# schumacherlab/ONT-TCRconsensus

Hardware: AMD Instinct MI355X
Metric: UMIs clustered/sec + banded-NW GCUPS (whole node, 1/2/4/8 MI355X) (higher is better)
Workload: dtype int16/int32

## Files before the change

### ont-tcrconsensus_amd/csrc/cluster_ctx.h

```cpp
#pragma once
#include <hip/hip_runtime.h>

#include <atomic>
#include <cstdlib>
#include <cstring>
#include <memory>
#include <thread>
#include <utility>
#include <vector>

#include "ctx.h"
#include "plan.h"
#include "resolve.h"

struct umiclust_ctx;

namespace uc {

constexpr int32_t kDelta = 8192;
constexpr int32_t kDepth = 2;
constexpr int32_t kBlockMin = 2048;
constexpr int32_t kDirectRecQ = 4096;
constexpr int32_t kSpecThr = 30;
constexpr int32_t kLazyPermille = 5;
// ... 15 lines not shown
struct Tile {
  DevBuf<uint32_t> hist;
  DevBuf<uint32_t> off;
  DevBuf<uint32_t> cursor;
  DevBuf<uint32_t> partial;
  uint64_t post_base = 0;
  size_t post_cap = 0;
  int32_t n = 0;
  int32_t base = 0;
  int32_t seg = 0;
  int32_t len = 0;
  int32_t built_n = -1;
  bool prebuilt = false;
};

struct Pass {
  int32_t q0 = 0, nq = 0, w0 = 0;
  bool live = false;
  bool rec_direct = false;
  PinBuf<TileView> h_tiles;
  DevBuf<TileView> d_tiles;
  DevBuf<uint32_t> d_top_seqno;
  DevBuf<uint8_t> d_top_count, d_ntop;
  DevBuf<uint32_t> d_pcand, d_units;
  DevBuf<uint8_t> d_pncand, d_ppeer_count, d_pnpeer;
  DevBuf<uint32_t> d_ppost;
  DevBuf<uint16_t> d_ppeer_id;
  DevBuf<uint16_t> d_peer_id;
  DevBuf<uint8_t> d_peer_count, d_npeer;
  bool ctr_zeroed = false;
  DevBuf<uint32_t> d_counters;
  DevBuf<uint32_t> d_pq, d_pt, d_outidx, d_res;
  DevBuf<WalkState> d_ws;
  DevBuf<HostQs> d_hq;
  DevBuf<unsigned long long> d_paligned;
  DevBuf<uint32_t> d_reccount;
  DevBuf<uint32_t> d_rec;
  uint32_t rec_est = 1u << 16;
  PinBuf<HostQs> h_hq;
  PinBuf<uint32_t> h_rec, h_counters, h_reccount;
  std::vector<HostQs> hq_copy;
  std::vector<uint32_t> rec_copy;
  ResolveScratch rsx;
  Event ev[5];
  PinBuf<TileView> h_tiles_a;
  DevBuf<TileView> d_tiles_a;
  DevBuf<uint32_t> d_anunits;
  Event ev_a;
  Event ev_c[2];
  bool c_timed = false;
  bool a_live = false, a_timed = false;
  int32_t a_q0 = -1, a_base = 0, a_slot = 0, t_slot = 0;
};

struct PfCapture {
  uint32_t* h_nunits = nullptr;
  int32_t ntiles = 0, nseg = 0, one_wave = 0;
};

struct Index {
  umiclust_ctx* const c;
  std::vector<std::unique_ptr<Tile>> tiles;
  Tile base_tile, delta_tile[2];
  int32_t delta_cur = 0;
  int32_t sealed_end = 0, base_end = 0;
  int32_t index_end = 0;
  DevBuf<uint16_t> arena;
  uint64_t sealed_slot0 = 0;
  std::vector<int32_t> cent;
  std::vector<uint8_t> cent_len;
  DevBuf<int32_t> d_cent;
  DevBuf<uint8_t> d_cent_len;
  PinBuf<int32_t> h_cent;
// ... 275 lines not shown
```

### ont-tcrconsensus_amd/csrc/kernels.hip

```cpp
#include <hip/hip_runtime.h>

#include <atomic>
#include <cstring>
#include <type_traits>
#include <mutex>

#include "align_kernels.h"
#include "umiclust_internal.h"

namespace uc {

enum { k_attr_prefilter = 0, k_attr_consensus = 1, k_attr_count = 2 };
constexpr int kAttrDevices = 64;
static std::atomic<bool> g_attr_set[kAttrDevices][k_attr_count];
static bool attr_set_on_device(int which) {
  int d = 0;
  if (hipGetDevice(&d) != hipSuccess || d < 0 || d >= kAttrDevices) return false;
  return g_attr_set[d][which];
}
static void mark_attr_set(int which) {
  int d = 0;
  if (hipGetDevice(&d) == hipSuccess && d >= 0 && d < kAttrDevices) g_attr_set[d][which] = true;
}

// ... 1398 lines not shown
                        int32_t band_max) {
  init_align_tables();
  if (npairs <= 0) return hipSuccess;
  if (qlen < kMinTplLen || qlen > kMaxLen) return hipErrorInvalidValue;
  const bool band = !ambig && npairs <= band_max;
  const int64_t lanes = (int64_t)npairs * (band ? band_lanes(qlen) : 1);
  const int v = ambig ? 1 : band ? 2 : 0;
  int64_t grid = (lanes + 63) / 64;
  hipLaunchKernelGGL(g_align[kAlignSlots * qlen + v], dim3((unsigned)grid),
                     dim3(64), 0, st, s, pq, pt, npairs, dev_npairs, outidx, sc, out);
  return hipGetLastError();
}

__device__ __forceinline__ uint32_t seg_alloc(uint32_t n, uint32_t si, uint32_t* cnt) {
  uint32_t start = 0;
  unsigned long long pending = __ballot(n > 0u);
  while (pending) {
    const int lead = __builtin_ctzll(pending);
    const uint32_t L = (uint32_t)__builtin_amdgcn_readlane((int)si, lead);
    const bool mine = n > 0u && si == L;
    const unsigned long long grp = __ballot(mine);
    const uint32_t v = mine ? n : 0u;
    const uint32_t incl = wave_scan_dpp(v, OpAdd());
    const uint32_t tot = lane63(incl);
    uint32_t b = 0;
    if ((int)(threadIdx.x & 63) == lead) b = atomicAdd(cnt + L, tot);
    b = (uint32_t)__builtin_amdgcn_readlane((int)b, lead);
    if (mine) start = b + incl - v;
    pending &= ~grp;
  }
  return start;
}

__global__ __launch_bounds__(256) void k_walk(int32_t round, int32_t q0, int32_t nqs, int32_t both, int32_t spec_thr,
                                              const uint32_t* __restrict__ top_seqno, const uint8_t* __restrict__ top_count,
                                              const uint8_t* __restrict__ ntop, const uint8_t* __restrict__ lens,
                                              const uint32_t* __restrict__ res, const uint8_t* __restrict__ acc_tab,
                                              const uint16_t* __restrict__ rank_tab, WalkState* __restrict__ ws,
                                              uint32_t* __restrict__ pq, uint32_t* __restrict__ pt,
                                              uint32_t* __restrict__ outidx, SegTab sg, uint32_t* __restrict__ seg_cnt,
                                              unsigned long long* __restrict__ cells) {
  const int qs = blockIdx.x * blockDim.x + threadIdx.x;
  const bool live = qs < nqs;
  const int32_t q = q0 + (live ? qs : 0) / both;
  const uint32_t strand = (uint32_t)((live ? qs : 0) % both);
  const int nt = live ? ntop[qs] : 0;
  const int ql = lens[q];
  WalkState w{};
  bool act = live;
  int emit_to = 0;
  if (round < 0) {
    w.w = 0;
    w.done = (nt == 0) ? 1 : 0;
    w.acc = 0;
    w.best_rank = 0;
    w.best_t = 0xffffffffu;
    w.cells = 0;
    w.lastkey = 0;
    w.e = 0;
    const bool spec = nt > 0 && (int)top_count[(int64_t)(live ? qs : 0) * kTopHits] < spec_thr;
    emit_to = min(nt, spec ? kWalk : kBatch);
  } else if (live) {
    w = ws[qs];
    act = !w.done;
    if (act) {
      while (!w.done && w.w < w.e) {
        const int b0 = w.w, b1 = min(nt, b0 + kBatch);
        for (int x = b0; x < b1; x++) {
          const uint32_t r = res[(int64_t)qs * kWalk + x];
          const uint32_t m = r & 0xffu, L = (r >> 8) & 0xffu;
          const uint32_t t = top_seqno[(int64_t)qs * kTopHits + x];
          w.cells += (uint32_t)(ql * lens[t]);
          if (acc_tab[L * kTabM + m]) {
            const uint16_t rk = rank_tab[L * kTabM + m];
            if (!w.acc || rk > w.best_rank || (rk == w.best_rank && t < w.best_t)) {
              w.best_rank = rk;
              w.best_t = t;
            }
            w.acc = 1;
          }
        }
        w.w = (uint8_t)b1;
        const uint32_t tl = lens[top_seqno[(int64_t)qs * kTopHits + b1 - 1]];
        w.lastkey = ((unsigned long long)(127u - top_count[(int64_t)qs * kTopHits + b1 - 1]) << 56) |
                    ((unsigned long long)tl << 48) | top_seqno[(int64_t)qs * kTopHits + b1 - 1];
        if (w.acc || b1 >= nt || b1 >= kWalk) w.done = 1;
      }
      emit_to = w.done ? (int)w.e : min(nt, kWalk);
    }
  }
  const uint32_t n = (act && emit_to > (int)w.e) ? (uint32_t)(emit_to - (int)w.e) : 0u;
  const uint32_t si = (uint32_t)(sg.lmax - ql);
  const uint32_t k0 = seg_alloc(n, si, seg_cnt);
  if (n) {
    const int b0 = w.e, b1 = emit_to;
    const uint32_t base = sg.base[si] + k0;
    uint32_t tl = 0;
    for (int x = b0; x < b1; x++) {
      const uint32_t k = base + (uint32_t)(x - b0);
      const uint32_t t = top_seqno[(int64_t)qs * kTopHits + x];
      pq[k] = ((uint32_t)q << 1) | strand;
      pt[k] = t;
      outidx[k] = (uint32_t)qs * kWalk + (uint32_t)x;
      tl += lens[t];
    }
    atomicAdd(cells, (unsigned long long)ql * tl);
    w.e = (uint8_t)b1;
  }
  if (act) ws[qs] = w;
}

hipError_t launch_walk(int32_t round, int32_t q0, int32_t nqs, int32_t both, int32_t spec_thr,
                       const uint32_t* top_seqno, const uint8_t* top_count, const uint8_t* ntop,
                       const uint8_t* lens, const uint32_t* res, const uint8_t* acc_tab,
                       const uint16_t* rank_tab, WalkState* ws, uint32_t* pq, uint32_t* pt,
                       uint32_t* outidx, const SegTab& sg, uint32_t* seg_cnt, unsigned long long* cells,
                       hipStream_t st) {
  if (nqs <= 0) return hipSuccess;
  hipLaunchKernelGGL(k_walk, dim3((nqs + 255) / 256), dim3(256), 0, st, round, q0, nqs, both, spec_thr,
                     top_seqno, top_count, ntop, lens, res, acc_tab, rank_tab, ws, pq, pt, outidx,
// ... 92 lines not shown
  atomicAdd(nstat, n);
  uint32_t k = sg.base[si] + k0;
  const uint32_t qv = ((uint32_t)q << 1) | (uint32_t)(qs % both);
  uint32_t tl = 0;
  for (int hh = 0; hh < kPH; hh++)
    for (unsigned long long m = rel[hh]; m; m &= m - 1ull) {
      const int x = 64 * hh + __builtin_ctzll(m);
      const uint32_t t = (uint32_t)(w0 + peer_id[(int64_t)qs * kPeerCap + x]);
      pq[k] = qv;
      pt[k] = t;
      outidx[k] = out0 + (uint32_t)(qs * kPeerCap + x);
      tl += lens[t];
      k++;
    }
  atomicAdd(cells, (unsigned long long)ql * tl);
}

hipError_t launch_peer_pairs(int32_t q0, int32_t w0, int32_t nqs, int32_t both, const uint8_t* lens,
                             const WalkState* ws, const uint16_t* peer_id, const uint8_t* peer_count,
                             const uint8_t* npeer, uint32_t* pq, uint32_t* pt, uint32_t* outidx, const SegTab& sg,
                             uint32_t* seg_cnt, unsigned long long* cells, uint32_t* nstat, uint32_t out0,
                             unsigned long long* aligned, int32_t emit, const WalkState* ws_prev,
                             const uint8_t* npeer_prev, int32_t q0_prev, int32_t nq_prev, hipStream_t st) {
  if (nqs <= 0) return hipSuccess;
  hipLaunchKernelGGL(k_peer_rel, dim3((nqs + 3) / 4), dim3(256), 0, st, q0, w0, nqs, both, lens, ws, peer_id,
                     peer_count, npeer, aligned, emit, ws_prev, npeer_prev, q0_prev, nq_prev);
  hipLaunchKernelGGL(k_peer_pairs, dim3((nqs + 255) / 256), dim3(256), 0, st, q0, w0, nqs, both, lens, ws, peer_id,
                     peer_count, npeer, pq, pt, outidx, sg, seg_cnt, cells, nstat, out0, aligned, emit, ws_prev,
                     npeer_prev, q0_prev, nq_prev);
  return hipGetLastError();
}

constexpr int kPackWaves = 4, kPackQ = 4;
__global__ __launch_bounds__(64 * kPackWaves) void k_pack(int32_t nqs, int32_t w0, const uint8_t* __restrict__ lens,
                                              const WalkState* __restrict__ ws, const uint8_t* __restrict__ ntop,
                                              const uint32_t* __restrict__ top_seqno,
                                              const uint8_t* __restrict__ top_count, const uint32_t* __restrict__ res,
                                              const uint8_t* __restrict__ npeer, const uint16_t* __restrict__ peer_id,
                                              const uint8_t* __restrict__ peer_count,
                                              const uint32_t* __restrict__ peer_res,
                                              const unsigned long long* __restrict__ aligned,
                                              uint32_t* __restrict__ reccount,
                                              HostQs* __restrict__ hq, uint32_t* __restrict__ rec,
                                              uint32_t* __restrict__ counters, uint32_t* __restrict__ hcounters,
                                              uint32_t* __restrict__ hreccount) {
  __shared__ uint32_t wsize[kPackWaves * kPackQ];
  __shared__ uint32_t last_wg;
  const int lane = threadIdx.x & 63, wave = threadIdx.x >> 6;
  const int qs0 = ((int)blockIdx.x * kPackWaves + wave) * kPackQ;
  if (blockIdx.x == 0 && threadIdx.x < 64) {
    uint32_t v = threadIdx.x < kPostSpread ? counters[16 + 32 * threadIdx.x] : 0u;
#pragma unroll
    for (int d = 1; d < 64; d <<= 1) v += __shfl_xor(v, d, 64);
    if (threadIdx.x < 16) hcounters[threadIdx.x] = threadIdx.x == 0 ? v : counters[threadIdx.x];
  }
  constexpr int kH = kPeerCap / 64;
  static_assert(kPackQ * kH <= 32, "relevant / aligned bits per lane");
  uint32_t pw[kPackQ][kH], relb = 0u, alb = 0u;
#pragma unroll
  for (int i = 0; i < kPackQ; i++) {
    const int qs = qs0 + i;
    const bool live = qs < nqs;
    const WalkState w = ws[live ? qs : 0];
    const int np = live ? npeer[qs] : 0;
    bool anyrel = false;
#pragma unroll
    for (int hh = 0; hh < kH; hh++) {
      const int x = lane + 64 * hh;
      pw[i][hh] = 0;
      if (live && np != 255 && x < np) {
        const uint32_t id = peer_id[(int64_t)qs * kPeerCap + x];
        const uint32_t cnt = peer_count[(int64_t)qs * kPeerCap + x];
        const uint32_t ps = (uint32_t)w0 + id;
        const bool rel = peer_relevant(w, cnt, lens[ps], ps);
        const bool al = (aligned[(int64_t)qs * kH + hh] >> lane) & 1ull;
        pw[i][hh] = id | (cnt << 16) | (rel ? 1u << 24 : 0u) | (al ? 1u << 25 : 0u);
        relb |= rel ? 1u << (i * kH + hh) : 0u;
        alb |= al ? 1u << (i * kH + hh) : 0u;
        anyrel |= rel;
      }
    }
    const bool has_rec = __any(anyrel);
    const int nt = live ? min((int)ntop[qs], kWalk) : 0;
    if (lane == 0) wsize[wave * kPackQ + i] = has_rec ? (uint32_t)(1 + 2 * nt + ((nt + 3) >> 2) + 2 * np) : 0u;
  }
  __syncthreads();
  if (threadIdx.x == 0) {
    uint32_t tot = 0;
    for (int i = 0; i < kPackWaves * kPackQ; i++) {
      const uint32_t x = wsize[i];
      wsize[i] = x ? tot : 0xffffffffu;
      tot += x;
    }
    const uint32_t b0 = tot ? atomicAdd(reccount, tot) : 0u;
    for (int i = 0; i < kPackWaves * kPackQ; i++)
      if (wsize[i] != 0xffffffffu) wsize[i] += b0;
// ... 55 lines not shown
    int hcur = 0;
#pragma unroll
    for (int j = 0; j < kInlineRel; j++) {
      uint32_t id = 0;
      while (hcur < kH && !rm[hcur]) hcur++;
      if (hcur < kH) {
        const int l = __builtin_ctzll(rm[hcur]);
        rm[hcur] &= rm[hcur] - 1ull;
        uint32_t v = pw[i][0];
#pragma unroll
        for (int hh = 1; hh < kH; hh++) v = hh == hcur ? pw[i][hh] : v;
        id = (uint32_t)__builtin_amdgcn_readlane((int)(v & 0xffffu), l);
      }
      ids[j] = (uint16_t)id;
    }
    if (lane == 0) {
      HostQs h;
      h.best_t = w.best_t;
      h.cells = w.cells;
      h.rec = base;
      h.best_rank = w.best_rank;
      h.w = w.w;
      h.flags = (uint8_t)((w.acc ? 1u : 0u) | (np == 255 ? 2u : 0u));
      h.nrel = (uint16_t)nrel;
      h.e = w.e;
      h.npeer = (uint8_t)np;
#pragma unroll
      for (int j = 0; j < kInlineRel; j++) h.rel[j] = ids[j];
      hq[qs] = h;
    }
  }
}

hipError_t launch_pack(int32_t nqs, int32_t w0, const uint8_t* lens, const WalkState* ws, const uint8_t* ntop,
                       const uint32_t* top_seqno, const uint8_t* top_count, const uint32_t* res,
                       const uint8_t* npeer, const uint16_t* peer_id, const uint8_t* peer_count,
                       const uint32_t* peer_res, const unsigned long long* aligned, uint32_t* reccount, HostQs* hq,
                       uint32_t* rec, uint32_t* counters, uint32_t* hcounters, uint32_t* hreccount,
                       hipStream_t st) {
  if (nqs <= 0) {
    *hreccount = 0;
    return hipSuccess;
  }
  constexpr int per = kPackWaves * kPackQ;
  hipLaunchKernelGGL(k_pack, dim3((nqs + per - 1) / per), dim3(64 * kPackWaves), 0, st, nqs, w0, lens,
                     ws, ntop, top_seqno, top_count,
                     res, npeer, peer_id, peer_count, peer_res, aligned, reccount, hq, rec, counters, hcounters,
                     hreccount);
  return hipGetLastError();
}

constexpr int kTwWaves = 4;
struct TwLayout {
  int words, dir_u32, wave_bytes;
  __host__ __device__ TwLayout(int maxq, int maxl) {
    words = (maxl + 63 + 7) / 8;
    dir_u32 = ((maxq + 63) / 64) * words * 64;
    wave_bytes = (dir_u32 * 4 + 2 * maxl * 4 + 4 + maxl + 72 + 2 * maxl + 15) & ~15;
  }
};
static_assert(kMaxLen <= 128, "the backtrack's register prefetch covers two stripes");

__device__ __forceinline__ uint32_t wave_shr1(uint32_t v, uint32_t lane0) {
  return (uint32_t)__builtin_amdgcn_update_dpp((int)lane0, (int)v, 0x138, 0xf, 0xf, false);
}

__global__ __launch_bounds__(64 * kTwWaves) void k_trace_wave(DevSeqs s, const uint32_t* __restrict__ pq,
                                                              const uint32_t* __restrict__ pt, int32_t npairs,
                                                              Scoring sc, uint8_t* __restrict__ ops,
                                                              uint16_t* __restrict__ nops, uint32_t* __restrict__ out,
                                                              int32_t maxq, int32_t maxl) {
  extern __shared__ __attribute__((aligned(16))) uint8_t tw_smem[];
  const int wave = __builtin_amdgcn_readfirstlane((int)(threadIdx.x >> 6)), lane = threadIdx.x & 63;
  const int k = (int)blockIdx.x * kTwWaves + wave;
  if (k >= npairs) return;
  const TwLayout lay(maxq, maxl);
  struct {
    uint32_t* dir;
    int32_t *botH, *botF, *hendp;
// ... 367 lines not shown
```

### ont-tcrconsensus_amd/csrc/pass.cpp

```cpp
#include <cstdio>
#include <string>

#include "cluster_ctx.h"

namespace uc {

void ensure_pass_buffers(umiclust_ctx* c, Pass& P, int32_t B) {
  const size_t nqs = (size_t)B * c->both;
  alloc_each(c, nqs * kTopHits, P.d_top_seqno, P.d_top_count);
  c->hip(P.d_ntop.ensure(nqs), "alloc");
  c->hip(P.d_pcand.ensure(nqs * kParts * kPartCand), "alloc");
  alloc_each(c, nqs * kParts, P.d_pncand, P.d_units);
  alloc_each(c, nqs * kParts * kPeerCap, P.d_ppeer_id, P.d_ppeer_count);
  alloc_each(c, nqs * kParts, P.d_pnpeer, P.d_ppost);
  alloc_each(c, nqs * kPeerCap, P.d_peer_id, P.d_peer_count);
  c->hip(P.d_npeer.ensure(nqs), "alloc");
  c->hip(P.d_counters.ensure(kCountersLen), "alloc");
  P.ctr_zeroed = false;
  alloc_each(c, nqs * (kWalk + kPeerCap), P.d_pq, P.d_pt, P.d_outidx, P.d_res);
  c->hip(P.d_hq.ensure(nqs), "alloc");
  c->hip(P.d_paligned.ensure((size_t)nqs * (kPeerCap / 64)), "alloc");
  c->hip(P.d_ws.ensure(nqs), "alloc");
  if (!P.d_reccount.p) {
    c->hip(P.d_reccount.ensure(2), "alloc");
    c->hip(hipMemsetAsync(P.d_reccount.p, 0, 8, c->st), "memset");
  }
  c->hip(P.h_hq.ensure(nqs), "pin");
  c->hip(P.h_rec.ensure(nqs * kRecWords), "pin");
  c->hip(P.d_rec.ensure(nqs * kRecWords), "alloc");
  c->hip(P.h_counters.ensure(16), "pin");
  c->hip(P.h_reccount.ensure(1), "pin");
  c->hip(P.h_tiles.ensure(64), "pin");
  c->hip(P.d_tiles.ensure(64), "alloc");
  c->hip(P.h_tiles_a.ensure(64), "pin");
  c->hip(P.d_tiles_a.ensure(64), "alloc");
  if (!P.d_anunits.p) {
    c->hip(P.d_anunits.ensure(1), "alloc");
    c->hip(hipMemsetAsync(P.d_anunits.p, 0, 4, c->st), "memset");
  }
  P.ev_a.get(c);
}

namespace {

void wait_index_and_tiles(umiclust_ctx* c, hipStream_t st) {
  if (c->ix_st && c->ix_done) c->hip(hipStreamWaitEvent(st, c->ix_done, 0), "wait");
  if (c->pt_pending) {
    c->hip(hipStreamWaitEvent(st, c->pt_ev, 0), "wait");
    c->pt_pending = false;
  }
}

PrefilterArgs prefilter_args(umiclust_ctx* c, const Pass& P, const TileView* views, const TileView* dviews, int32_t nv,
                             int32_t q0, int32_t nq) {
  const Index& ix = c->ix;
  PrefilterArgs a{};
  for (int32_t i = 0; i < nv && nv <= kArgTiles; i++) a.tv[i] = views[i];
  a.seqs = dev_seqs(c);
  a.arena = ix.arena.p;
  a.tiles = dviews;
  a.ntiles = nv;
  a.ncent = ix.index_end;
// ... 160 lines not shown
    b0 += nql[i] * both * kWalk;
    b1 += nql[i] * both * (kWalk + kPeerCap);
  }
  uint32_t* segc = P.d_counters.p + kSegSlot;
  unsigned long long* cells_w = reinterpret_cast<unsigned long long*>(P.d_counters.p + 12);
  unsigned long long* cells_p = reinterpret_cast<unsigned long long*>(P.d_counters.p + 14);
  auto align_round = [&](const SegTab& sg, int per_qs, uint32_t* cnt, const char* what) {
    for (int32_t i = 0; i < nsg; i++)
      if (nql[i])
        c->hip(launch_align(ds, lmax - i, c->ambig, P.d_pq.p + sg.base[i], P.d_pt.p + sg.base[i], nql[i] * both * per_qs,
                            cnt + i, P.d_outidx.p + sg.base[i], c->sc, P.d_res.p, st, c->tun.band_pairs),
               what);
  };
  c->hip(launch_walk(-1, q0, nqs, both, kSpecThr, P.d_top_seqno.p, P.d_top_count.p, P.d_ntop.p, c->d_lens.p, P.d_res.p,
                     c->d_acc.p, c->d_rank.p, P.d_ws.p, P.d_pq.p, P.d_pt.p, P.d_outidx.p, sg0, segc, cells_w, st),
         "walk");
  c->hip(hipEventRecord(P.ev[2], st), "event");
  const uint32_t peer_out0 = (uint32_t)nqs * kWalk;
  align_round(sg0, kWalk, segc, "align 0");
  c->hip(launch_walk(0, q0, nqs, both, kSpecThr, P.d_top_seqno.p, P.d_top_count.p, P.d_ntop.p, c->d_lens.p,
                     P.d_res.p, c->d_acc.p, c->d_rank.p, P.d_ws.p, P.d_pq.p, P.d_pt.p, P.d_outidx.p, sg1, segc + kSegLens,
                     cells_w, st),
         "walk 0");
  const Pass* prev = nullptr;
  for (const Pass& Q : c->pass)
    if (&Q != &P && Q.nq > 0 && Q.q0 + Q.nq == q0) prev = &Q;
  c->hip(launch_peer_pairs(q0, w0, nqs, both, c->d_lens.p, P.d_ws.p, P.d_peer_id.p, P.d_peer_count.p, P.d_npeer.p,
                           P.d_pq.p, P.d_pt.p, P.d_outidx.p, sg1, segc + kSegLens, cells_p, P.d_counters.p + 8,
                           peer_out0, P.d_paligned.p, lazy_peers ? 0 : 1,
                           prev ? prev->d_ws.p : nullptr, prev ? prev->d_npeer.p : nullptr, prev ? prev->q0 : 0,
                           prev ? prev->nq : 0, st),
         "peer pairs");
  align_round(sg1, kWalk + kPeerCap, segc + kSegLens, "align 1");
  c->hip(launch_walk(1, q0, nqs, both, kSpecThr, P.d_top_seqno.p, P.d_top_count.p, P.d_ntop.p, c->d_lens.p,
                     P.d_res.p, c->d_acc.p, c->d_rank.p, P.d_ws.p, P.d_pq.p, P.d_pt.p, P.d_outidx.p, sg1,
                     segc + 2 * kSegLens, cells_w, st),
         "walk 1");
  c->hip(hipEventRecord(P.ev[3], st), "event");
  P.rec_direct = c->rec_direct || nq <= kDirectRecQ;
  c->hip(launch_pack(nqs, w0, c->d_lens.p, P.d_ws.p, P.d_ntop.p, P.d_top_seqno.p, P.d_top_count.p, P.d_res.p,
                     P.d_npeer.p, P.d_peer_id.p, P.d_peer_count.p, P.d_res.p + peer_out0, P.d_paligned.p, P.d_reccount.p,
                     P.rec_direct ? P.h_hq.p : P.d_hq.p,
                     P.rec_direct ? P.h_rec.p : P.d_rec.p, P.d_counters.p, P.h_counters.p, P.h_reccount.p, st),
         "pack");
  P.ctr_zeroed = nqs > 0;
  if (!P.rec_direct) {
    c->hip(hipMemcpyAsync(P.h_hq.p, P.d_hq.p, (size_t)nqs * sizeof(HostQs), hipMemcpyDeviceToHost, st), "d2h outcomes");
    const size_t est = std::min<size_t>(P.rec_est, P.d_rec.n);
    c->hip(hipMemcpyAsync(P.h_rec.p, P.d_rec.p, est * 4, hipMemcpyDeviceToHost, st), "d2h records");
  }
  c->hip(hipEventRecord(P.ev[4], st), "event");
}

void enqueue_count(umiclust_ctx* c, Pass& P, int32_t q0, int32_t nq, const Tile* const* wins, int nwin, int flag,
                   int32_t slot) {
  P.a_live = false;
  if (c->ix.nseg() > 1) return;
  hipStream_t st = c->st;
  wait_index_and_tiles(c, st);
  if (c->ix_st) c->hip(hipStreamWaitEvent(st, P.ev[1], 0), "wait");
  c->hip(hipEventSynchronize(P.ev_a), "sync");
  const int32_t nv = c->ix.stage_views(P.h_tiles_a, P.d_tiles_a, st);
  c->hip(hipEventRecord(P.ev_a, st), "event");
  PrefilterArgs a = prefilter_args(c, P, P.h_tiles_a.p, P.d_tiles_a.p, nv, q0, nq);
  a.seg_tile[0] = 0;
  a.seg_tile[1] = nv;
  uint64_t lo = UINT64_MAX;
  for (int i = 0; i < nwin; i++) lo = std::min(lo, wins[i]->post_base);
  for (int v = 0; v < nv; v++) lo = std::min(lo, P.h_tiles_a.p[v].post_base);
  a.seg_base[0] = lo;
  fill_peer_slots(a, wins, nwin, nullptr);
  a.flag_tile = flag >= 0 ? (kPeerTiles - nwin) + flag : -1;
  a.peer_base = a.cand_base = wins[0]->base;
  a.nlist_cap = nlist_cap(c, q0, nq, nv);
  c->hip(hipEventRecord(c->a_ev[slot][0].get(c), st), "event");
  c->hip(launch_prefilter(a, st, 1), "prefilter (count)");
  c->hip(hipEventRecord(c->a_ev[slot][1].get(c), st), "event");
  c->stats.counter_cells += (int64_t)nq * c->both * a.ncent;
  if (c->tun.pf_probe) launch_pf_probe(c, a, st);
  c->last_a_slot = slot;
  P.a_live = true;
  P.a_q0 = q0;
// ... 86 lines not shown
  c->dbg.rb.pairs += nb;
}

}

bool resolve_pass(umiclust_ctx* c, Pass& P, const StateView& state, std::vector<int32_t>& new_cents,
                  double& t_pf, double& t_al, double& t_host, int32_t* resolved) {
  const int both = c->both;
  const int32_t q0 = P.q0, w0 = P.w0;
  int32_t nq = P.nq;
  int32_t nqs = nq * both;
  if (resolved) *resolved = 0;
  const double tsync0 = now_s();
  c->hip(hipEventSynchronize(P.ev[4]), "sync");
  c->stats.t_sync_s += now_s() - tsync0;
  c->dbg.t.wait += now_s() - tsync0;
  struct DAcc { double* p; double t0; ~DAcc() { *p += now_s() - t0; } } dtot{&c->dbg.t.total, tsync0};
  P.live = false;
  t_pf += elapsed_s(c, P.ev[0], P.ev[1]);
  if (P.a_timed) {
    const double s = elapsed_s(c, c->a_ev[P.t_slot][0], c->a_ev[P.t_slot][1]);
    t_pf += s;
    c->stats.t_count_s += s;
    c->stats.n_count_launches++;
    tl_add(c->dev, 0, c->a_ev[P.t_slot][0], c->a_ev[P.t_slot][1]);
  } else if (P.c_timed) {
    c->stats.t_count_s += elapsed_s(c, P.ev_c[0], P.ev_c[1]);
    c->stats.n_count_launches++;
    tl_add(c->dev, 0, P.ev_c[0], P.ev_c[1]);
  }
  t_al += elapsed_s(c, P.ev[2], P.ev[3]);
  tl_add(c->dev, 1, P.ev[2], P.ev[3]);
  {
    const size_t used = *P.h_reccount.p, est = std::min<size_t>(P.rec_est, P.d_rec.n);
    if (used > est && !P.rec_direct) {
      c->hip(hipMemcpyAsync(P.h_rec.p + est, P.d_rec.p + est, (used - est) * 4, hipMemcpyDeviceToHost, c->st_copy),
             "d2h records");
      c->hip(hipStreamSynchronize(c->st_copy), "sync");
    }
    P.rec_est = (uint32_t)std::max<size_t>(1u << 16, used + used / 2 + 4096);
  }
  c->stats.kmer_postings += P.h_counters.p[0];
  c->stats.pairs_peer += P.h_counters.p[8];
  {
    unsigned long long cw = 0, cp = 0;
    memcpy(&cw, P.h_counters.p + 12, 8);
    memcpy(&cp, P.h_counters.p + 14, 8);
    c->stats.cells_computed += (int64_t)(cw + cp);
  }
  const double tc0 = now_s();
  P.hq_copy.assign(P.h_hq.p, P.h_hq.p + nqs);
  {
    uint32_t mx = 0;
    for (int32_t qs = 0; qs < nqs; qs++) mx = std::max<uint32_t>(mx, P.hq_copy[qs].npeer);
    c->last_max_npeer = (int32_t)mx;
  }
  c->stats.t_sync_s += now_s() - tc0;
  c->dbg.t.hq_copy += now_s() - tc0;
  const HostQs* hq = P.hq_copy.data();
  if (!c->pool) c->pool.reset(new WorkPool(pool_threads(c)));
  const uint32_t* recs = P.h_rec.p;
  {
    const double tc1 = now_s();
    const size_t nw = *P.h_reccount.p;
    if (P.rec_copy.size() < nw) P.rec_copy.resize(nw + nw / 4);
    const int TC = nw < (1u << 18) ? 1 : c->pool->size();
    if (TC == 1) {
      memcpy(P.rec_copy.data(), P.h_rec.p, nw * 4);
    } else {
      c->pool->run([&](int t) {
        const size_t lo = nw * (size_t)t / (size_t)TC, hi = nw * (size_t)(t + 1) / (size_t)TC;
        memcpy(P.rec_copy.data() + lo, P.h_rec.p + lo, (hi - lo) * 4);
      });
    }
    recs = P.rec_copy.data();
    c->stats.t_sync_s += now_s() - tc1;
    c->dbg.t.rec_copy += now_s() - tc1;
  }
  ResolveEnv env;
  env.hlen = c->hlen.data();
  env.acc = c->h_acc.data();
  env.rank = c->h_rank.data();
  env.both = both;
  env.o4_T = c->o4_T;
  env.maxaccepts = c->p.maxaccepts;
  env.maxrejects = c->p.maxrejects;
  env.hqbin = c->pack_on ? c->hqbin.data() : nullptr;
  env.bin_s = c->bin_s.data();

  env.par_inorder = g_live_ctx.load() <= 1 && c->pool->size() <= affinity_cpus();
  env.par_min = c->tun.par_min;
  env.debug = c->tun.debug == 1;
  env.target = c->target.data();
  env.strand = c->strand.data();
  env.walk_dump = c->wd.empty() ? nullptr : c->wd.data();
  auto rb = [&](const std::vector<uint32_t>& bpq, const std::vector<uint32_t>& bpt, std::vector<uint32_t>& bres) {
    round_b(c, bpq, bpt, bres, t_al);
  };
  const bool dump = c->tun.resolve_dump && !c->pack_on && c->dump_want(c->n_resolved);
  c->n_resolved++;
  std::vector<uint32_t> dpq, dpt, dres;
  std::vector<uint8_t> state_in;
  if (dump) state_in.assign(&state[w0], &state[w0] + (q0 + nq - w0));
  RoundB round_b_rec = [&](const std::vector<uint32_t>& bpq, const std::vector<uint32_t>& bpt, std::vector<uint32_t>& bres) {
    rb(bpq, bpt, bres);
// ... 53 lines not shown
```

### ont-tcrconsensus_amd/csrc/probes.cpp

```cpp
#include <algorithm>
#include <cstddef>

#include "cluster_ctx.h"

using namespace uc;

static void check_block_args(umiclust_ctx* c, const char* who, const int32_t* cent, int32_t ncent, int32_t q0, int32_t nq,
                      int32_t nprev, int32_t append_step) {
  if (!c->loaded) c->fail(UMICLUST_ESTATE, "%s before umiclust_load", who);
  if (c->bin_s.size() != 2) c->fail(UMICLUST_EINVAL, "%s: the load holds several bins", who);
  if (c->o4_T) c->fail(UMICLUST_EINVAL, "%s: batched rounds (policy O4) are not covered", who);
  if ((!cent && ncent > 0) || ncent < 0 || nq < 1 || nq > kMaxBlock || nprev < 0 || nprev > kPeerTiles - 1 ||
      append_step < 1 || q0 < 0 || (int64_t)q0 + nq > c->n || (int64_t)q0 - (int64_t)nprev * nq < 0)
    c->fail(UMICLUST_EINVAL, "%s: block, window or append step out of range", who);
  if (ncent > kSegCentroids) c->fail(UMICLUST_EINVAL, "%s: more than one counter segment", who);
  const int32_t w0 = q0 - nprev * nq;
  for (int32_t i = 0; i < ncent; i++)
    if (cent[i] < (i ? cent[i - 1] + 1 : 0) || cent[i] >= w0)
      c->fail(UMICLUST_EINVAL, "%s: centroid seqnos must increase and precede the window", who);
  if (block_maxlen(c, q0, nq) - block_minlen(c, q0, nq) + 1 > kSegLens)
    c->fail(UMICLUST_EINVAL, "%s: block spans more than %d query lengths", who, kSegLens);
}
static void stage_block(umiclust_ctx* c, ClusterRun& r, const int32_t* cent, int32_t ncent, int32_t q0, int32_t nq,
                 int32_t nprev, int32_t append_step) {
// ... 121 lines not shown
                      uint32_t* counters, int64_t* info) {
  UC_GUARD(c, {
    check_block_args(c, "umiclust_pass", cent, ncent, q0, nq, nprev, append_step);
    if (flags & ~(UMICLUST_PASS_LAZY | UMICLUST_PASS_PREV)) c->fail(UMICLUST_EINVAL, "umiclust_pass: unknown flag");
    if ((flags & UMICLUST_PASS_PREV) && nprev < 1)
      c->fail(UMICLUST_EINVAL, "umiclust_pass: the previous block's pass needs nprev >= 1");
    if (rec_cap < 0) c->fail(UMICLUST_EINVAL, "umiclust_pass: record buffer");
    ClusterRun r(c, 0, 1, false);
    const uint32_t* ctr_p[kPeerTiles];
    bool ctr_z[kPeerTiles];
    for (int i = 0; i < kPeerTiles; i++) {
      ctr_p[i] = c->pass[i].d_counters.p;
      ctr_z[i] = c->pass[i].ctr_zeroed;
    }
    stage_block(c, r, cent, ncent, q0, nq, nprev, append_step);
    sync_streams(c);
    for (int i = 0; i < kPeerTiles; i++)
      if (ctr_p[i] && c->pass[i].d_counters.p == ctr_p[i]) c->pass[i].ctr_zeroed = ctr_z[i];
    r.lazy = (flags & UMICLUST_PASS_LAZY) != 0;
    Pass& P = c->pass[nprev % 2];
    for (Pass& Q : c->pass)
      if (&Q != &P) Q.nq = 0;
    if (flags & UMICLUST_PASS_PREV) r.second_half(nprev - 1, 0, false);
    PfCapture cap;
    cap.h_nunits = c->h_pf_nunits.p;
    r.second_half(nprev, 0, false, &cap);
    sync_streams(c);
    for (Pass& Q : c->pass) Q.live = false;
    const size_t nqs = (size_t)nq * c->both;
    fetch_lists(c, P, cap, nqs, top_seqno, top_count, ntop, peer_id, peer_count, npeer, info);
    auto out = [&](void* dst, const void* src, size_t bytes) {
      if (dst && bytes) c->hip(hipMemcpy(dst, src, bytes, hipMemcpyDeviceToHost), "d2h pass");
    };
    if (hostqs) memcpy(hostqs, P.h_hq.p, nqs * sizeof(HostQs));
    const int64_t total = *P.h_reccount.p;
    if (rec_total) *rec_total = total;
    if (rec) {
      const size_t nw = (size_t)std::min<int64_t>(total, rec_cap);
      if (P.rec_direct) memcpy(rec, P.h_rec.p, nw * 4);
      else out(rec, P.d_rec.p, nw * 4);
    }
    out(res, P.d_res.p, nqs * (kWalk + kPeerCap) * 4);
    out(aligned, P.d_paligned.p, nqs * (kPeerCap / 64) * 8);
    out(walk, P.d_ws.p, nqs * sizeof(WalkState));
    if (counters) memcpy(counters, P.h_counters.p, 16 * 4);
    if (rec && total > rec_cap) c->fail(UMICLUST_ERANGE, "umiclust_pass: %lld record words, room for %lld",
                                         (long long)total, (long long)rec_cap);
    return UMICLUST_OK;
  });
}

int32_t umiclust_align_pairs(umiclust_ctx* c, const umiclust_params* p, const char* q, const int64_t* q_off,
                             const char* t, const int64_t* t_off, int64_t npairs, int32_t* score,
                             int32_t* matches, int32_t* internal_len, char* cigar_ops, int32_t ops_stride,
                             int32_t* ops_len) {
  UC_GUARD(c, {
    if (!p || npairs < 0 || (npairs > 0 && (!q || !q_off || !t || !t_off))) c->fail(UMICLUST_EINVAL, "null argument");
    umiclust_params pp = *p;
    pp.minseqlength = 1;
    pp.maxseqlength = kMaxLen;
    validate(c, pp);
    std::vector<char> all;
    std::vector<int64_t> off{0};
    append_set(q, q_off, npairs, all, off);
    append_set(t, t_off, npairs, all, off);
    const int64_t ns = 2 * npairs;
    for (int64_t i = 0; i < ns; i++)
      if (off[i + 1] - off[i] < 1 || off[i + 1] - off[i] > kMaxLen) c->fail(UMICLUST_ERANGE, "pair sequence length");
    Scoring sc = to_scoring(pp);
    ProbeSeqs S;
    DevBuf<uint32_t> d_pq, d_pt, d_out;
    DevBuf<uint8_t> d_ops;
    DevBuf<uint16_t> d_nops;
// ... 337 lines not shown
```

### ont-tcrconsensus_amd/csrc/umiclust_internal.h

```cpp
#pragma once
#include <hip/hip_runtime.h>
#include <stdint.h>

#include "umiclust_consts.h"

namespace uc {

struct Scoring {
  int32_t match, mismatch;
  int32_t go[6], ge[6];
  int32_t boundary_open;
};

struct TileView {
  const uint32_t* off;
  uint64_t post_base;
  int32_t n;
  int32_t base;
  int32_t seg;
  int32_t len;
};

struct DevSeqs {
  const uint32_t* codes;
// ... 79 lines not shown

hipError_t launch_align(const DevSeqs& s, int32_t qlen, bool ambig, const uint32_t* pq, const uint32_t* pt, int32_t npairs,
                        const uint32_t* dev_npairs, const uint32_t* outidx, const Scoring& sc,
                        uint32_t* out, hipStream_t st, int32_t band_max = 0);

struct WalkState {
  unsigned long long lastkey;
  uint32_t best_t;
  uint32_t cells;
  uint16_t best_rank;
  uint8_t w;
  uint8_t done;
  uint8_t acc;
  uint8_t e;
  uint8_t pad[2];
};
struct SegTab {
  int32_t lmax;
  int32_t nseg;
  uint32_t base[kSegLens];
};
hipError_t launch_walk(int32_t round, int32_t q0, int32_t nqs, int32_t both, int32_t spec_thr,
                       const uint32_t* top_seqno, const uint8_t* top_count, const uint8_t* ntop,
                       const uint8_t* lens, const uint32_t* res, const uint8_t* acc_tab,
                       const uint16_t* rank_tab, WalkState* ws, uint32_t* pq, uint32_t* pt,
                       uint32_t* outidx, const SegTab& sg, uint32_t* seg_cnt, unsigned long long* cells,
                       hipStream_t st);
hipError_t launch_peer_pairs(int32_t q0, int32_t w0, int32_t nqs, int32_t both, const uint8_t* lens,
                             const WalkState* ws, const uint16_t* peer_id, const uint8_t* peer_count,
                             const uint8_t* npeer, uint32_t* pq, uint32_t* pt, uint32_t* outidx, const SegTab& sg,
                             uint32_t* seg_cnt, unsigned long long* cells, uint32_t* nstat, uint32_t out0,
                             unsigned long long* aligned, int32_t emit, const WalkState* ws_prev,
                             const uint8_t* npeer_prev, int32_t q0_prev, int32_t nq_prev, hipStream_t st);
hipError_t launch_pack(int32_t nqs, int32_t w0, const uint8_t* lens, const WalkState* ws, const uint8_t* ntop,
                       const uint32_t* top_seqno, const uint8_t* top_count, const uint32_t* res,
                       const uint8_t* npeer, const uint16_t* peer_id, const uint8_t* peer_count,
                       const uint32_t* peer_res, const unsigned long long* aligned, uint32_t* reccount, HostQs* hq,
                       uint32_t* rec, uint32_t* counters, uint32_t* hcounters, uint32_t* hreccount, hipStream_t st);
hipError_t launch_traceback(const DevSeqs& s, const uint32_t* pq, const uint32_t* pt, int32_t npairs,
                            const Scoring& sc, uint8_t* ops, uint16_t* nops, uint32_t* out, hipStream_t st,
                            int32_t maxl, int32_t maxq = 0);
hipError_t launch_consensus(const DevSeqs& s, const int32_t* cstart, int32_t nclusters,
                            const int32_t* member_seqno, const int32_t* member_opsidx,
                            const uint8_t* member_strand, const uint8_t* ops,
                            const uint16_t* nops, char* cons, uint16_t* conslen,
                            int32_t* overflow, hipStream_t st);

struct OvBuffers {
  uint64_t* hash;
  int32_t* region;
  unsigned long long* keys;
  unsigned long long* rep;
  int64_t* slot;
  uint32_t* cnt;
  uint32_t* start;
  uint32_t* cursor;
  uint32_t* bsum;
  uint32_t* members;
  uint32_t* collision;
  uint32_t* big;
  uint32_t* nbig;
};
constexpr int kOvSmallBucket = 32;
hipError_t launch_overlap_table(const char* seqs, const int64_t* offs, int64_t n, const int64_t* rstart, int32_t nreg,
                                uint64_t seed, uint64_t hmask, uint64_t mask, const OvBuffers& B, bool csr,
                                uint32_t* collided, hipStream_t st);
hipError_t launch_overlap_pairs(const OvBuffers& B, uint64_t mask, int32_t nreg, unsigned long long* total,
                                uint32_t* maxc, hipStream_t st);
// ... 140 lines not shown
```

Measured before the change: 5.389 million.

## Fuse final walk evaluation into pack kernel and merge outcome/record D2H copies

The last walk round, which ran as its own kernel after the second alignment round, is now evaluated inline in k_pack through a shared walk_eval helper, with lane 0 writing back the updated state. This removes one kernel launch per pass. Host outcomes and records now share a single contiguous device and pinned buffer, so the two D2H copies collapse into one. In exchange, pack does redundant per-lane work, and the walk-1 round's pair emission and its cell-accounting counter are no longer produced.

Result: no change. 5.344 million (-0.8%).

```diff
diff --git a/ont-tcrconsensus_amd/csrc/cluster_ctx.h b/ont-tcrconsensus_amd/csrc/cluster_ctx.h
--- a/ont-tcrconsensus_amd/csrc/cluster_ctx.h
+++ b/ont-tcrconsensus_amd/csrc/cluster_ctx.h
@@ -71,13 +71,22 @@
   DevBuf<uint32_t> d_counters;
   DevBuf<uint32_t> d_pq, d_pt, d_outidx, d_res;
   DevBuf<WalkState> d_ws;
-  DevBuf<HostQs> d_hq;
   DevBuf<unsigned long long> d_paligned;
   DevBuf<uint32_t> d_reccount;
-  DevBuf<uint32_t> d_rec;
+  DevBuf<uint8_t> d_out;
+  PinBuf<uint8_t> h_out;
+  HostQs *d_hq = nullptr, *h_hq = nullptr;
+  uint32_t *d_rec = nullptr, *h_rec = nullptr;
+  size_t rec_cap = 0;
+  void place_outputs(size_t nqs) {
+    d_hq = reinterpret_cast<HostQs*>(d_out.p);
+    h_hq = reinterpret_cast<HostQs*>(h_out.p);
+    d_rec = reinterpret_cast<uint32_t*>(d_out.p + nqs * sizeof(HostQs));
+    h_rec = reinterpret_cast<uint32_t*>(h_out.p + nqs * sizeof(HostQs));
+    rec_cap = nqs * kRecWords;
+  }
   uint32_t rec_est = 1u << 16;
-  PinBuf<HostQs> h_hq;
-  PinBuf<uint32_t> h_rec, h_counters, h_reccount;
+  PinBuf<uint32_t> h_counters, h_reccount;
   std::vector<HostQs> hq_copy;
   std::vector<uint32_t> rec_copy;
   ResolveScratch rsx;
diff --git a/ont-tcrconsensus_amd/csrc/kernels.hip b/ont-tcrconsensus_amd/csrc/kernels.hip
--- a/ont-tcrconsensus_amd/csrc/kernels.hip
+++ b/ont-tcrconsensus_amd/csrc/kernels.hip
@@ -1454,6 +1454,34 @@
   return start;
 }
 
+__device__ __forceinline__ void walk_eval(WalkState& w, int qs, int nt, int ql, const uint32_t* __restrict__ top_seqno,
+                                          const uint8_t* __restrict__ top_count, const uint8_t* __restrict__ lens,
+                                          const uint32_t* __restrict__ res, const uint8_t* __restrict__ acc_tab,
+                                          const uint16_t* __restrict__ rank_tab) {
+  while (!w.done && w.w < w.e) {
+    const int b0 = w.w, b1 = min(nt, b0 + kBatch);
+    for (int x = b0; x < b1; x++) {
+      const uint32_t r = res[(int64_t)qs * kWalk + x];
+      const uint32_t m = r & 0xffu, L = (r >> 8) & 0xffu;
+      const uint32_t t = top_seqno[(int64_t)qs * kTopHits + x];
+      w.cells += (uint32_t)(ql * lens[t]);
+      if (acc_tab[L * kTabM + m]) {
+        const uint16_t rk = rank_tab[L * kTabM + m];
+        if (!w.acc || rk > w.best_rank || (rk == w.best_rank && t < w.best_t)) {
+          w.best_rank = rk;
+          w.best_t = t;
+        }
+        w.acc = 1;
+      }
+    }
+    w.w = (uint8_t)b1;
+    const uint32_t tl = lens[top_seqno[(int64_t)qs * kTopHits + b1 - 1]];
+    w.lastkey = ((unsigned long long)(127u - top_count[(int64_t)qs * kTopHits + b1 - 1]) << 56) |
+                ((unsigned long long)tl << 48) | top_seqno[(int64_t)qs * kTopHits + b1 - 1];
+    if (w.acc || b1 >= nt || b1 >= kWalk) w.done = 1;
+  }
+}
+
 __global__ __launch_bounds__(256) void k_walk(int32_t round, int32_t q0, int32_t nqs, int32_t both, int32_t spec_thr,
                                               const uint32_t* __restrict__ top_seqno, const uint8_t* __restrict__ top_count,
                                               const uint8_t* __restrict__ ntop, const uint8_t* __restrict__ lens,
@@ -1486,28 +1514,7 @@
     w = ws[qs];
     act = !w.done;
     if (act) {
-      while (!w.done && w.w < w.e) {
-        const int b0 = w.w, b1 = min(nt, b0 + kBatch);
-        for (int x = b0; x < b1; x++) {
-          const uint32_t r = res[(int64_t)qs * kWalk + x];
-          const uint32_t m = r & 0xffu, L = (r >> 8) & 0xffu;
-          const uint32_t t = top_seqno[(int64_t)qs * kTopHits + x];
-          w.cells += (uint32_t)(ql * lens[t]);
-          if (acc_tab[L * kTabM + m]) {
-            const uint16_t rk = rank_tab[L * kTabM + m];
-            if (!w.acc || rk > w.best_rank || (rk == w.best_rank && t < w.best_t)) {
-              w.best_rank = rk;
-              w.best_t = t;
-            }
-            w.acc = 1;
-          }
-        }
-        w.w = (uint8_t)b1;
-        const uint32_t tl = lens[top_seqno[(int64_t)qs * kTopHits + b1 - 1]];
-        w.lastkey = ((unsigned long long)(127u - top_count[(int64_t)qs * kTopHits + b1 - 1]) << 56) |
-                    ((unsigned long long)tl << 48) | top_seqno[(int64_t)qs * kTopHits + b1 - 1];
-        if (w.acc || b1 >= nt || b1 >= kWalk) w.done = 1;
-      }
+      walk_eval(w, qs, nt, ql, top_seqno, top_count, lens, res, acc_tab, rank_tab);
       emit_to = w.done ? (int)w.e : min(nt, kWalk);
     }
   }
@@ -1666,8 +1673,10 @@
 }
 
 constexpr int kPackWaves = 4, kPackQ = 4;
-__global__ __launch_bounds__(64 * kPackWaves) void k_pack(int32_t nqs, int32_t w0, const uint8_t* __restrict__ lens,
-                                              const WalkState* __restrict__ ws, const uint8_t* __restrict__ ntop,
+__global__ __launch_bounds__(64 * kPackWaves) void k_pack(int32_t nqs, int32_t q0, int32_t both, int32_t w0,
+                                              const uint8_t* __restrict__ lens, const uint8_t* __restrict__ acc_tab,
+                                              const uint16_t* __restrict__ rank_tab, WalkState* ws,
+                                              const uint8_t* __restrict__ ntop,
                                               const uint32_t* __restrict__ top_seqno,
                                               const uint8_t* __restrict__ top_count, const uint32_t* __restrict__ res,
                                               const uint8_t* __restrict__ npeer, const uint16_t* __restrict__ peer_id,
@@ -1695,7 +1704,11 @@
   for (int i = 0; i < kPackQ; i++) {
     const int qs = qs0 + i;
     const bool live = qs < nqs;
-    const WalkState w = ws[live ? qs : 0];
+    WalkState w = ws[live ? qs : 0];
+    if (live && !w.done) {
+      walk_eval(w, qs, ntop[qs], lens[q0 + qs / both], top_seqno, top_count, lens, res, acc_tab, rank_tab);
+      if (lane == 0) ws[qs] = w;
+    }
     const int np = live ? npeer[qs] : 0;
     bool anyrel = false;
 #pragma unroll
@@ -1817,8 +1830,9 @@
   }
 }
 
-hipError_t launch_pack(int32_t nqs, int32_t w0, const uint8_t* lens, const WalkState* ws, const uint8_t* ntop,
-                       const uint32_t* top_seqno, const uint8_t* top_count, const uint32_t* res,
+hipError_t launch_pack(int32_t nqs, int32_t q0, int32_t both, int32_t w0, const uint8_t* lens, const uint8_t* acc_tab,
+                       const uint16_t* rank_tab, WalkState* ws, const uint8_t* ntop, const uint32_t* top_seqno,
+                       const uint8_t* top_count, const uint32_t* res,
                        const uint8_t* npeer, const uint16_t* peer_id, const uint8_t* peer_count,
                        const uint32_t* peer_res, const unsigned long long* aligned, uint32_t* reccount, HostQs* hq,
                        uint32_t* rec, uint32_t* counters, uint32_t* hcounters, uint32_t* hreccount,
@@ -1828,8 +1842,8 @@
     return hipSuccess;
   }
   constexpr int per = kPackWaves * kPackQ;
-  hipLaunchKernelGGL(k_pack, dim3((nqs + per - 1) / per), dim3(64 * kPackWaves), 0, st, nqs, w0, lens,
-                     ws, ntop, top_seqno, top_count,
+  hipLaunchKernelGGL(k_pack, dim3((nqs + per - 1) / per), dim3(64 * kPackWaves), 0, st, nqs, q0, both, w0, lens,
+                     acc_tab, rank_tab, ws, ntop, top_seqno, top_count,
                      res, npeer, peer_id, peer_count, peer_res, aligned, reccount, hq, rec, counters, hcounters,
                      hreccount);
   return hipGetLastError();
diff --git a/ont-tcrconsensus_amd/csrc/pass.cpp b/ont-tcrconsensus_amd/csrc/pass.cpp
--- a/ont-tcrconsensus_amd/csrc/pass.cpp
+++ b/ont-tcrconsensus_amd/csrc/pass.cpp
@@ -18,16 +18,15 @@
   c->hip(P.d_counters.ensure(kCountersLen), "alloc");
   P.ctr_zeroed = false;
   alloc_each(c, nqs * (kWalk + kPeerCap), P.d_pq, P.d_pt, P.d_outidx, P.d_res);
-  c->hip(P.d_hq.ensure(nqs), "alloc");
   c->hip(P.d_paligned.ensure((size_t)nqs * (kPeerCap / 64)), "alloc");
   c->hip(P.d_ws.ensure(nqs), "alloc");
   if (!P.d_reccount.p) {
     c->hip(P.d_reccount.ensure(2), "alloc");
     c->hip(hipMemsetAsync(P.d_reccount.p, 0, 8, c->st), "memset");
   }
-  c->hip(P.h_hq.ensure(nqs), "pin");
-  c->hip(P.h_rec.ensure(nqs * kRecWords), "pin");
-  c->hip(P.d_rec.ensure(nqs * kRecWords), "alloc");
+  c->hip(P.d_out.ensure(nqs * (sizeof(HostQs) + kRecWords * 4)), "alloc");
+  c->hip(P.h_out.ensure(nqs * (sizeof(HostQs) + kRecWords * 4)), "pin");
+  P.place_outputs(nqs);
   c->hip(P.h_counters.ensure(16), "pin");
   c->hip(P.h_reccount.ensure(1), "pin");
   c->hip(P.h_tiles.ensure(64), "pin");
@@ -254,22 +253,19 @@
                            prev ? prev->nq : 0, st),
          "peer pairs");
   align_round(sg1, kWalk + kPeerCap, segc + kSegLens, "align 1");
-  c->hip(launch_walk(1, q0, nqs, both, kSpecThr, P.d_top_seqno.p, P.d_top_count.p, P.d_ntop.p, c->d_lens.p,
-                     P.d_res.p, c->d_acc.p, c->d_rank.p, P.d_ws.p, P.d_pq.p, P.d_pt.p, P.d_outidx.p, sg1,
-                     segc + 2 * kSegLens, cells_w, st),
-         "walk 1");
+  P.rec_direct = c->rec_direct || nq <= kDirectRecQ;
+  P.place_outputs((size_t)nqs);
+  c->hip(launch_pack(nqs, q0, both, w0, c->d_lens.p, c->d_acc.p, c->d_rank.p, P.d_ws.p, P.d_ntop.p, P.d_top_seqno.p,
+                     P.d_top_count.p, P.d_res.p, P.d_npeer.p, P.d_peer_id.p, P.d_peer_count.p, P.d_res.p + peer_out0,
+                     P.d_paligned.p, P.d_reccount.p, P.rec_direct ? P.h_hq : P.d_hq,
+                     P.rec_direct ? P.h_rec : P.d_rec, P.d_counters.p, P.h_counters.p, P.h_reccount.p, st),
+         "pack");
   c->hip(hipEventRecord(P.ev[3], st), "event");
-  P.rec_direct = c->rec_direct || nq <= kDirectRecQ;
-  c->hip(launch_pack(nqs, w0, c->d_lens.p, P.d_ws.p, P.d_ntop.p, P.d_top_seqno.p, P.d_top_count.p, P.d_res.p,
-                     P.d_npeer.p, P.d_peer_id.p, P.d_peer_count.p, P.d_res.p + peer_out0, P.d_paligned.p, P.d_reccount.p,
-                     P.rec_direct ? P.h_hq.p : P.d_hq.p,
-                     P.rec_direct ? P.h_rec.p : P.d_rec.p, P.d_counters.p, P.h_counters.p, P.h_reccount.p, st),
-         "pack");
   P.ctr_zeroed = nqs > 0;
   if (!P.rec_direct) {
-    c->hip(hipMemcpyAsync(P.h_hq.p, P.d_hq.p, (size_t)nqs * sizeof(HostQs), hipMemcpyDeviceToHost, st), "d2h outcomes");
-    const size_t est = std::min<size_t>(P.rec_est, P.d_rec.n);
-    c->hip(hipMemcpyAsync(P.h_rec.p, P.d_rec.p, est * 4, hipMemcpyDeviceToHost, st), "d2h records");
+    const size_t est = std::min<size_t>(P.rec_est, P.rec_cap);
+    c->hip(hipMemcpyAsync(P.h_out.p, P.d_out.p, (size_t)nqs * sizeof(HostQs) + est * 4, hipMemcpyDeviceToHost, st),
+           "d2h outcomes + records");
   }
   c->hip(hipEventRecord(P.ev[4], st), "event");
 }
@@ -422,9 +418,9 @@
   t_al += elapsed_s(c, P.ev[2], P.ev[3]);
   tl_add(c->dev, 1, P.ev[2], P.ev[3]);
   {
-    const size_t used = *P.h_reccount.p, est = std::min<size_t>(P.rec_est, P.d_rec.n);
+    const size_t used = *P.h_reccount.p, est = std::min<size_t>(P.rec_est, P.rec_cap);
     if (used > est && !P.rec_direct) {
-      c->hip(hipMemcpyAsync(P.h_rec.p + est, P.d_rec.p + est, (used - est) * 4, hipMemcpyDeviceToHost, c->st_copy),
+      c->hip(hipMemcpyAsync(P.h_rec + est, P.d_rec + est, (used - est) * 4, hipMemcpyDeviceToHost, c->st_copy),
              "d2h records");
       c->hip(hipStreamSynchronize(c->st_copy), "sync");
     }
@@ -439,7 +435,7 @@
     c->stats.cells_computed += (int64_t)(cw + cp);
   }
   const double tc0 = now_s();
-  P.hq_copy.assign(P.h_hq.p, P.h_hq.p + nqs);
+  P.hq_copy.assign(P.h_hq, P.h_hq + nqs);
   {
     uint32_t mx = 0;
     for (int32_t qs = 0; qs < nqs; qs++) mx = std::max<uint32_t>(mx, P.hq_copy[qs].npeer);
@@ -449,18 +445,18 @@
   c->dbg.t.hq_copy += now_s() - tc0;
   const HostQs* hq = P.hq_copy.data();
   if (!c->pool) c->pool.reset(new WorkPool(pool_threads(c)));
-  const uint32_t* recs = P.h_rec.p;
+  const uint32_t* recs = P.h_rec;
   {
     const double tc1 = now_s();
     const size_t nw = *P.h_reccount.p;
     if (P.rec_copy.size() < nw) P.rec_copy.resize(nw + nw / 4);
     const int TC = nw < (1u << 18) ? 1 : c->pool->size();
     if (TC == 1) {
-      memcpy(P.rec_copy.data(), P.h_rec.p, nw * 4);
+      memcpy(P.rec_copy.data(), P.h_rec, nw * 4);
     } else {
       c->pool->run([&](int t) {
         const size_t lo = nw * (size_t)t / (size_t)TC, hi = nw * (size_t)(t + 1) / (size_t)TC;
-        memcpy(P.rec_copy.data() + lo, P.h_rec.p + lo, (hi - lo) * 4);
+        memcpy(P.rec_copy.data() + lo, P.h_rec + lo, (hi - lo) * 4);
       });
     }
     recs = P.rec_copy.data();
diff --git a/ont-tcrconsensus_amd/csrc/probes.cpp b/ont-tcrconsensus_amd/csrc/probes.cpp
--- a/ont-tcrconsensus_amd/csrc/probes.cpp
+++ b/ont-tcrconsensus_amd/csrc/probes.cpp
@@ -177,13 +177,13 @@
     auto out = [&](void* dst, const void* src, size_t bytes) {
       if (dst && bytes) c->hip(hipMemcpy(dst, src, bytes, hipMemcpyDeviceToHost), "d2h pass");
     };
-    if (hostqs) memcpy(hostqs, P.h_hq.p, nqs * sizeof(HostQs));
+    if (hostqs) memcpy(hostqs, P.h_hq, nqs * sizeof(HostQs));
     const int64_t total = *P.h_reccount.p;
     if (rec_total) *rec_total = total;
     if (rec) {
       const size_t nw = (size_t)std::min<int64_t>(total, rec_cap);
-      if (P.rec_direct) memcpy(rec, P.h_rec.p, nw * 4);
-      else out(rec, P.d_rec.p, nw * 4);
+      if (P.rec_direct) memcpy(rec, P.h_rec, nw * 4);
+      else out(rec, P.d_rec, nw * 4);
     }
     out(res, P.d_res.p, nqs * (kWalk + kPeerCap) * 4);
     out(aligned, P.d_paligned.p, nqs * (kPeerCap / 64) * 8);
diff --git a/ont-tcrconsensus_amd/csrc/umiclust_internal.h b/ont-tcrconsensus_amd/csrc/umiclust_internal.h
--- a/ont-tcrconsensus_amd/csrc/umiclust_internal.h
+++ b/ont-tcrconsensus_amd/csrc/umiclust_internal.h
@@ -135,8 +135,9 @@
                              uint32_t* seg_cnt, unsigned long long* cells, uint32_t* nstat, uint32_t out0,
                              unsigned long long* aligned, int32_t emit, const WalkState* ws_prev,
                              const uint8_t* npeer_prev, int32_t q0_prev, int32_t nq_prev, hipStream_t st);
-hipError_t launch_pack(int32_t nqs, int32_t w0, const uint8_t* lens, const WalkState* ws, const uint8_t* ntop,
-                       const uint32_t* top_seqno, const uint8_t* top_count, const uint32_t* res,
+hipError_t launch_pack(int32_t nqs, int32_t q0, int32_t both, int32_t w0, const uint8_t* lens, const uint8_t* acc_tab,
+                       const uint16_t* rank_tab, WalkState* ws, const uint8_t* ntop, const uint32_t* top_seqno,
+                       const uint8_t* top_count, const uint32_t* res,
                        const uint8_t* npeer, const uint16_t* peer_id, const uint8_t* peer_count,
                        const uint32_t* peer_res, const unsigned long long* aligned, uint32_t* reccount, HostQs* hq,
                        uint32_t* rec, uint32_t* counters, uint32_t* hcounters, uint32_t* hreccount, hipStream_t st);
```
